# zovoilis-lab/Flye

Hardware: AMD Instinct MI355X
Metric: Gbp reads overlapped/sec (higher is better)
Workload: dtype u64

## Files before the change

### flye_amd/csrc/fg_chain.hip

```cpp
#include "fg_wavesort.h"

#include <algorithm>

#define WG 256
#define I32_MIN ((i32)0x80000000)

struct ChainParams {
	int k, maxJump, minOverlap, maxOverhang;
	int checkOverhang, forceLocal;
	float minUnique;
	u32 firstId;
	u32 qFirstId;
	int onlyMaxExt;
	int keepAln;
	int ablate;
	int lazy;
	unsigned long long* lazyCnt;
};

namespace {

struct CandAcc {
	typedef int4 T;
	int4* c;
	__device__ int4 load(int i) const { return c[i]; }
	__device__ void store(int i, const int4& x) { c[i] = x; }
	__device__ bool less(const int4& a, const int4& b) const { return a.w > b.w; }
};

__device__ __forceinline__ bool overlap_test(const ChainParams& P, u32 curId, u32 extId, i32 curLen,
											 i32 extLen, i32 cb, i32 ce, i32 eb, i32 ee)
{
	const i32 curRange = ce - cb, extRange = ee - eb;
	if (curRange < P.minOverlap || extRange < P.minOverlap) return false;
	const float lengthDiff = (float)abs(curRange - extRange);
	if (lengthDiff > 0.5f * (float)min(curRange, extRange)) return false;
	if (curId == extId)
	{
		const i32 inter = min(ce, ee) - max(cb, eb);
		if (inter > curRange / 2) return false;
	}
	if (curId == (extId ^ 1u))
	{
		const i32 inter = min(ce, extLen - eb) - max(cb, extLen - ee);
		if (inter > curRange / 2) return false;
	}
	if (!P.forceLocal && P.checkOverhang)
	{
		const i32 ovh = max(min(cb, eb), min(curLen - ce, extLen - ee));
		if (ovh > P.maxOverhang) return false;
	}
	return true;
}

#define LIST_ITEMS 8
__device__ __forceinline__ void append2_multi(const bool (&a)[LIST_ITEMS], const bool (&b)[LIST_ITEMS], u32 g0,
											  u32* listA, u32* listB, u32* counts)
{
	__shared__ u32 wtot[2][WG / 64];
	__shared__ u32 base[2];
	const int lane = threadIdx.x & 63, wv = threadIdx.x >> 6;
	u32 cA = 0, cB = 0;
#pragma unroll
	for (int t = 0; t < LIST_ITEMS; ++t) { cA += a[t]; cB += b[t]; }
	u32 iA = cA, iB = cB;
	for (int o = 1; o < 64; o <<= 1)
	{
		const u32 x = __shfl_up(iA, o), y = __shfl_up(iB, o);
		if (lane >= o) { iA += x; iB += y; }
	}
	if (lane == 63) { wtot[0][wv] = iA; wtot[1][wv] = iB; }
	__syncthreads();
	if (threadIdx.x < 2)
	{
		u32 t = 0;
		for (int i = 0; i < WG / 64; ++i) t += wtot[threadIdx.x][i];
		base[threadIdx.x] = t ? atomicAdd(&counts[threadIdx.x], t) : 0u;
	}
	__syncthreads();
	u32 oA = base[0] + iA - cA, oB = base[1] + iB - cB;
	for (int i = 0; i < wv; ++i) { oA += wtot[0][i]; oB += wtot[1][i]; }
#pragma unroll
	for (int t = 0; t < LIST_ITEMS; ++t)
	{
		if (a[t]) listA[oA++] = g0 + (u32)t;
		if (b[t]) listB[oB++] = g0 + (u32)t;
	}
}

__global__ void k_group_list(u64 nGroups, u64 nHits, const u64* __restrict__ groupStart, u32 minSize,
							 const u32* __restrict__ groupFirstCur, const u32* __restrict__ groupLastCur, i32 minOverlap,
							 u32* __restrict__ list, u32* __restrict__ listBig, u32 bigMin,
							 u32* __restrict__ listFused, u32 fusedMax , u32* __restrict__ counts,
							 u32* __restrict__ primCount, u32* __restrict__ dpSize)
{
	const u64 g0 = ((u64)blockIdx.x * WG + threadIdx.x) * LIST_ITEMS;
	bool a[LIST_ITEMS], b[LIST_ITEMS], f[LIST_ITEMS], none[LIST_ITEMS];
	u64 start = g0 < nGroups ? groupStart[g0] : nHits;
#pragma unroll
	for (int t = 0; t < LIST_ITEMS; ++t)
	{
		const u64 g = g0 + t;
		u64 n = 0;
		bool ok = false;
		if (g < nGroups)
		{
			primCount[g] = 0;
			dpSize[g] = 0;
			const u64 gend = (g + 1 < nGroups) ? groupStart[g + 1] : nHits;
			n = gend - start;
			if (n >= minSize && n > 0)
				ok = (i32)groupLastCur[g] - (i32)groupFirstCur[g] >= minOverlap;
			start = gend;
		}
		f[t] = ok && n <= fusedMax;
		a[t] = ok && n > fusedMax && n <= bigMin;
		b[t] = ok && n > bigMin && n > fusedMax;
		none[t] = false;
	}
	append2_multi(a, b, (u32)g0, list, listBig, counts);
	if (fusedMax)
	{
		__syncthreads();
		append2_multi(f, none, (u32)g0, listFused, listFused, counts + 2);
	}
}

#ifndef FIN_CAP_S
#define FIN_CAP_S 256
#endif
#ifndef FIN_CAP_M
#define FIN_CAP_M 1024
#endif
#ifndef FIN_WAVES_S
#define FIN_WAVES_S 1
#endif
#ifndef FIN_WAVES_G
#define FIN_WAVES_G 1
#endif
#ifndef FIN_BT_CAP
#define FIN_BT_CAP 1024
#endif
__global__ void k_dp_list(u64 nGroups, const u32* __restrict__ dpSize, u32 hugeMin, u32 doneMax ,
						  u32* __restrict__ listSmall, u32* __restrict__ listMid, u32* __restrict__ listBig, u32* __restrict__ counts)
{
	const u64 g0 = ((u64)blockIdx.x * WG + threadIdx.x) * LIST_ITEMS;
	bool a[LIST_ITEMS], b[LIST_ITEMS], h[LIST_ITEMS], none[LIST_ITEMS];
#pragma unroll
	for (int t = 0; t < LIST_ITEMS; ++t)
	{
		const u32 n = g0 + t < nGroups ? dpSize[g0 + t] : 0u;
		a[t] = n > doneMax && n <= FIN_CAP_S;
		b[t] = n > FIN_CAP_S && n > doneMax && n <= hugeMin;
		h[t] = n > hugeMin && n > FIN_CAP_S && n > doneMax;
		none[t] = false;
	}
	append2_multi(a, b, (u32)g0, listSmall, listMid, counts);
	__syncthreads();
	append2_multi(h, none, (u32)g0, listBig, listBig, counts + 2);
}

#ifndef PREP_CAP
#define PREP_CAP 320
#endif
#ifndef PREP_WAVES
#define PREP_WAVES 1
#endif
template <class KT>
__global__ void __launch_bounds__(PREP_WAVES * 64)
k_group_prep(ChainParams P, const u32* __restrict__ list, u32 nList, u64 nGroups, u64 nHits,
			 const u64* __restrict__ groupStart, const u32* __restrict__ groupQuery,
			 const u32* __restrict__ query, const i32* __restrict__ len, const i32* __restrict__ qLen,
			 HitKeyView<KT> hitKey, const u32* __restrict__ groupExt,
			 u32* __restrict__ gCur, u32* __restrict__ gExt, u32* __restrict__ gAux ,
			 u32* __restrict__ dpSize, uint8_t* __restrict__ groupExtSorted)
{
	__shared__ u32 sExt[PREP_WAVES][PREP_CAP];
// ... 197 lines not shown
				}
				const i32 j = jb - lane;
				i32 cp = FAR, ep = FAR, sj = 0;
				if (j >= 0)
				{
					if (WHOLE) { cp = (i32)cur[j]; ep = (i32)ext[j]; sj = score[j]; }
					else if (j >= tb0 - DP_RING)
					{
						cp = ringC[j & (DP_RING - 1)]; ep = ringE[j & (DP_RING - 1)]; sj = ringS[j & (DP_RING - 1)];
					}
					else
					{
						__builtin_amdgcn_s_waitcnt(0);
						cp = (i32)cur[j]; ep = (i32)ext[j];
						sj = __hip_atomic_load(&score[j], __ATOMIC_RELAXED, __HIP_MEMORY_SCOPE_AGENT);
					}
				}
				const i32 dc = cn - cp, de = en - ep;
				const bool inr = max((u32)(dc - 1), (u32)(de - 1)) < (u32)(maxJump - 1);
				const i32 jd = (i32)abs_diff(dc, de);
				i32 nsRaw = sj + min(min(dc, de), k) - (jd > 100 ? 2 * jd : (jd >> 1));
				asm volatile("" : "+v"(nsRaw));
				const i32 ns = inr ? nsRaw : I32_MIN;
				const u64 inrM = __builtin_amdgcn_ballot_w64(inr);
				const u64 mB = __builtin_amdgcn_ballot_w64((EXTS ? de : dc) > maxJump);
				const u64 mA = __builtin_amdgcn_ballot_w64(dc == de) & __builtin_amdgcn_ballot_w64(dc < k) & inrM;
				done = dp_scan_step(ns, mA, __popcll(~mB), jb, maxScore, maxId);
			}
			const i32 sNew = max(maxScore, k);
			ts = hl == il ? sNew + off : ts;
			tbk = lane == il ? (maxScore > k ? maxId : -1) : tbk;
		}
		asm volatile("" : "+v"(ntc), "+v"(nte));
		if (valid)
		{
			score[tb0 + lane] = ts; back[tb0 + lane] = tbk;
			if (!WHOLE) { ringC[(tb0 + lane) & (DP_RING - 1)] = tc; ringE[(tb0 + lane) & (DP_RING - 1)] = te; ringS[(tb0 + lane) & (DP_RING - 1)] = ts; }
		}
		if (WHOLE) wsort::wave_mem_fence();
		{
			const i32 tileMax = __builtin_amdgcn_readlane(wave_incl_max(valid ? ts : I32_MIN), 63);
			pmRun = max(pmRun, tileMax);
			const int t = tb0 >> 6;
			if (t < 64) pmv = lane == t ? pmRun : pmv;
		}
		pc = tc; pe = te; ps = ts;
	}
}

__global__ void __launch_bounds__(DP_WAVES * 64)
k_chain_dp(ChainParams P, const u32* __restrict__ list, u32 nList, u64 nGroups, u64 nHits,
		   const u64* __restrict__ groupStart, const u32* __restrict__ groupQuery,
		   const u32* __restrict__ query, const i32* __restrict__ len, const i32* __restrict__ qLen,
		   const uint8_t* __restrict__ groupExtSorted,
		   const u32* __restrict__ gCur, const u32* __restrict__ gExt,
		   i32* __restrict__ gScore, i32* __restrict__ gBack)
{
	const u32 li = blockIdx.x * DP_WAVES + (threadIdx.x >> 6);
	if (li >= nList) return;
	const u64 g = fg_uni(list[li]);
	const u64 g0 = fg_uni(groupStart[g]);
	const u64 gend = (g + 1 < nGroups) ? fg_uni(groupStart[g + 1]) : nHits;
	const i32 n = (i32)(gend - g0);
	const bool extSorted = fg_uni((u32)groupExtSorted[g]) != 0;
	__shared__ i32 ring[DP_WAVES][3][DP_RING];
	i32* ringC = ring[threadIdx.x >> 6][0];
	i32* ringE = ring[threadIdx.x >> 6][1];
	i32* ringS = ring[threadIdx.x >> 6][2];
	if (extSorted) dp_group<true>(P.k, P.maxJump, n, gCur + g0, gExt + g0, gScore + g0, gBack + g0, ringC, ringE, ringS);
	else dp_group<false>(P.k, P.maxJump, n, gCur + g0, gExt + g0, gScore + g0, gBack + g0, ringC, ringE, ringS);
}

template <int R>
__device__ __forceinline__ i32 fast_score_order(const i32 n, const i32* score, const i32* back, u32* oval)
{
	const int lane = threadIdx.x & 63;
	u32 v[R];
	bool wide = false;
#pragma unroll
	for (int r = 0; r < R; ++r)
	{
		const i32 e = r * 64 + lane;
		const bool live = e < n && back[e] != -1;
		const i32 sc = live ? score[e] : 0;
		wide |= live && (u32)sc >= (1u << 22);
		v[r] = live ? ((u32)((1 << 22) - 1 - sc) << 10) | (u32)e : 0xFFFFFFFFu;
	}
	if (__builtin_amdgcn_ballot_w64(wide)) return -1;
#pragma unroll
	for (int k = 2; k <= 64 * R; k <<= 1)
	{
#pragma unroll
		for (int j = k >> 1; j > 0; j >>= 1)
		{
			if (j >= 64)
			{
#pragma unroll
				for (int r = 0; r < R; ++r)
				{
					const int rp = r ^ (j >> 6);
					if (rp > r)
					{
						const bool asc = ((r * 64) & k) == 0;
						const u32 lo = min(v[r], v[rp]), hi = max(v[r], v[rp]);
						v[r] = asc ? lo : hi; v[rp] = asc ? hi : lo;
					}
				}
			}
			else
			{
#pragma unroll
				for (int r = 0; r < R; ++r)
				{
// ... 271 lines not shown
				m &= __builtin_amdgcn_ballot_w64(bk2 != -1);
			}
		}
	}
	wsort::wave_mem_fence();
	if (lane != 0) return;
	if (ncand == 0) return;
	if (ncand > 16)
	{
		CandAcc acc{cd};
		fgsort::sort(acc, 0, ncand, stack);
		best = cd[0];
	}
	if (P.onlyMaxExt)
	{
		cd[0] = best;
		*primCountG = 1;
		return;
	}
	if (ncand <= 16)
		for (i32 a = 1; a < ncand; ++a)
		{
			const int4 v = cd[a];
			i32 b = a - 1;
			while (b >= 0 && cd[b].w < v.w) { cd[b + 1] = cd[b]; --b; }
			cd[b + 1] = v;
		}
	i32 nprim = 0;
	for (i32 a = 0; a < ncand; ++a)
	{
		const int4 o = cd[a];
		const i32 ocb = (i32)cur[o.x], oce = (i32)cur[o.y], oeb = (i32)ext[o.x], oee = (i32)ext[o.y];
		bool contained = false;
		for (i32 b = 0; b < nprim && !contained; ++b)
		{
			const int4 pr = cd[b];
			contained = pr.w > o.w && (i32)cur[pr.x] <= ocb && oce <= (i32)cur[pr.y] &&
						(i32)ext[pr.x] <= oeb && oee <= (i32)ext[pr.y];
		}
		if (!contained) cd[nprim++] = o;
	}
	*primCountG = (u32)nprim;
}


template <int CAP, int FIN_WAVES, int BT_CAP = 0>
__global__ void __launch_bounds__(FIN_WAVES * 64)
k_chain_finish(ChainParams P, const u32* __restrict__ list, u32 nList, u64 nGroups, u64 nHits,
			   const u64* __restrict__ groupStart, const u32* __restrict__ groupQuery,
			   const u32* __restrict__ query, const i32* __restrict__ len, const i32* __restrict__ qLen,
			   const u32* __restrict__ groupExt,
			   const u32* __restrict__ gCur, const u32* __restrict__ gExt, i32* __restrict__ gScore,
			   i32* __restrict__ gBack, u32* __restrict__ gAux , int4* __restrict__ cand,
			   u32* __restrict__ primCount)
{
	constexpr bool USE_LDS = CAP > 0;
	extern __shared__ __attribute__((aligned(16))) char finLds[];
	__shared__ int stack[FIN_WAVES][3 * 40];
	__shared__ int small[FIN_WAVES][3 * 8];
	__shared__ i32 btLds[FIN_WAVES][BT_CAP > 0 ? BT_CAP : 1];
	const int wv = threadIdx.x >> 6;
	const int lane = threadIdx.x & 63;
	const u32 li = blockIdx.x * FIN_WAVES + wv;
	if (li >= nList) return;
	const u64 g = fg_uni(list[li]);
	const u64 g0 = fg_uni(groupStart[g]);
	const u64 gend = (g + 1 < nGroups) ? fg_uni(groupStart[g + 1]) : nHits;
	const i32 n = (i32)(gend - g0);
	const u32 q = groupQuery[g];
	const u32* cur = gCur + g0;
	const u32* ext = gExt + g0;
	i32 *score, *back; u32 *okey, *oval;
	unsigned short* plLds = nullptr;
	if (USE_LDS)
	{
		char* base = finLds + (size_t)wv * CAP * 20;
		score = (i32*)base; back = score + CAP; okey = (u32*)(back + CAP); oval = okey + CAP;
		plLds = (unsigned short*)(oval + CAP);
		for (i32 i = lane; i < n; i += 64) { score[i] = gScore[g0 + i]; back[i] = gBack[g0 + i]; }
		wsort::wave_mem_fence();
	}
	else
	{
		score = gScore + g0; back = gBack + g0; okey = gAux + 4 * g0; oval = okey + n;
	}
	const u32 qrec = query[q];
	const u32 extId = groupExt[g];
	finish_group<USE_LDS, BT_CAP>(P, n, P.qFirstId + qrec, extId, qLen[qrec >> 1], len[(extId - P.firstId) >> 1], cur, ext, score, back,
								  okey, oval, plLds, stack[wv], small[wv], btLds[wv], cand + g0, primCount + g);
}

template <class KT>
__global__ void __launch_bounds__(64)
k_chain_small(ChainParams P, const u32* __restrict__ list, u32 nList, u64 nGroups, u64 nHits,
			  const u64* __restrict__ groupStart, const u32* __restrict__ groupQuery,
			  const u32* __restrict__ query, const i32* __restrict__ len, const i32* __restrict__ qLen,
			  HitKeyView<KT> hitKey, const u32* __restrict__ groupExt,
			  u32* __restrict__ gCur, u32* __restrict__ gExt, i32* __restrict__ gBack, int4* __restrict__ cand,
			  u32* __restrict__ dpSize, u32* __restrict__ primCount, int cap )
{
	extern __shared__ __attribute__((aligned(16))) char smallLds[];
	u32* const sCur = (u32*)smallLds; u32* const sExt = sCur + cap;
	i32* const sScore = (i32*)(sExt + cap); i32* const sBack = sScore + cap;
	u32* const sOkey = (u32*)(sBack + cap); u32* const sOval = sOkey + cap;
	unsigned short* const sP = (unsigned short*)(sOval + cap);
	__shared__ int stack[3 * 40];
	__shared__ int small[3 * 8];
	const int lane = threadIdx.x;
	const u32 li = blockIdx.x;
	if (li >= nList) return;
	const u64 g = fg_uni(list[li]);
	const u64 g0 = fg_uni(groupStart[g]);
	const u64 gend = (g + 1 < nGroups) ? fg_uni(groupStart[g + 1]) : nHits;
	const i32 n = (i32)(gend - g0);
	const u32 qrec = query[groupQuery[g]];
	const u32 extId = groupExt[g];
	const i32 curLen = qLen[qrec >> 1];
	const i32 extLen = len[(extId - P.firstId) >> 1];
// ... 32 lines not shown
		if (__builtin_amdgcn_ballot_w64(!asc))
			wsort::wave_sort<u32, unsigned short>(sExt, sCur, n, sP, sP + n, stack, small);
	}
	for (i32 i = lane; i < n; i += 64) { gCur[g0 + i] = sCur[i]; gExt[g0 + i] = sExt[i]; }
	wsort::wave_mem_fence();
	if (extSorted) dp_group<true, true>(P.k, P.maxJump, n, sCur, sExt, sScore, sBack, nullptr, nullptr, nullptr);
	else dp_group<false, true>(P.k, P.maxJump, n, sCur, sExt, sScore, sBack, nullptr, nullptr, nullptr);
	wsort::wave_mem_fence();
	if (P.keepAln)
		for (i32 i = lane; i < n; i += 64) gBack[g0 + i] = sBack[i];
	finish_group<true, 0>(P, n, P.qFirstId + qrec, extId, curLen, extLen, sCur, sExt, sScore, sBack, sOkey, sOval, sP, stack, small,
						  nullptr, cand + g0, primCount + g);
}

u32 fetchU32(fg_ctx* c, const u32* dptr)
{
	u32 v;
	HIP_CHECK(hipMemcpyAsync(&v, dptr, 4, hipMemcpyDeviceToHost, c->stream));
	HIP_CHECK(hipStreamSynchronize(c->stream));
	return v;
}

}

u32 fgChainSmallMax()
{
	if (getenv("FG_CHAIN_FUSED") && atoi(getenv("FG_CHAIN_FUSED")) == 0) return 0u;
	return getenv("FG_FUSED_CAP") ? (u32)std::max(64, std::min(1024, atoi(getenv("FG_FUSED_CAP")))) : (u32)FIN_CAP_S;
}

void fgChainStage(fg_ctx* c, const fg_detector_params* p, uint8_t forceLocal, u64 nGroups, u64 nHits, int keyMode,
				  int curBits)
{
	hipStream_t s = c->stream;
	ChainParams cp;
	cp.k = c->k; cp.maxJump = p->max_jump; cp.minOverlap = p->min_overlap; cp.maxOverhang = p->max_overhang;
	cp.checkOverhang = p->max_overhang > 0; cp.forceLocal = forceLocal ? 1 : 0;
	{
		const float minKmerSruvivalRate = 0.01;
		cp.minUnique = minKmerSruvivalRate * p->min_overlap;
	}
	cp.firstId = c->firstId;
	cp.qFirstId = c->hasQ ? c->qFirstId : c->firstId;
	cp.onlyMaxExt = p->only_max_ext ? 1 : 0;
	cp.keepAln = p->keep_alignment ? 1 : 0;
	cp.ablate = getenv("FG_ABLATE") ? atoi(getenv("FG_ABLATE")) : 0;
	cp.lazy = cp.onlyMaxExt && !(getenv("FG_CHAIN_LAZY") && atoi(getenv("FG_CHAIN_LAZY")) == 0);
	cp.lazyCnt = c->dLazyCnt.p;
	if (!nGroups) return;
	const i32* qLen = c->hasQ ? c->dQLen.p : c->dLen.p;
	u32 minSize = 0;
	while ((float)minSize < cp.minUnique) ++minSize;
	if (minSize == 0) minSize = 1;
	c->dListSmall.reserve(nGroups + 1); c->dListBig.reserve(nGroups + 1); c->dListDp.reserve(nGroups + 1);
	c->dGroupExtSorted.reserve(nGroups + 1);
	c->dListCnt.reserve(4);
	const u64 hitCap = std::max<u64>(nHits, c->hitCapHint);
	c->dCur.reserve(hitCap + 16); c->dExt.reserve(hitCap + 16);
	c->dScore.reserve(hitCap + 16); c->dBack.reserve(hitCap + 16);
	c->dTmp32.reserve(4 * hitCap + 16);
	c->dCand.reserve(hitCap + 1);
	const unsigned gridG = (unsigned)((nGroups + (u64)WG * LIST_ITEMS - 1) / ((u64)WG * LIST_ITEMS));
	const u32 fusedMax = fgChainSmallMax();
	const bool fused = fusedMax != 0;
	if (fused) c->dListFused.reserve(nGroups + 1);
	HIP_CHECK(hipMemsetAsync(c->dListCnt.p, 0, 16, s));
	{ ScopedK t(c->timer, "k_group_list");
	  hipLaunchKernelGGL(k_group_list, gridG, WG, 0, s, nGroups, nHits, c->dGroupStart.p, minSize, c->dGroupFirstCur.p,
						 c->dGroupLastCur.p, (i32)p->min_overlap, c->dListSmall.p, c->dListBig.p, (u32)PREP_CAP,
						 c->dListFused.p, fusedMax, c->dListCnt.p, c->dPrimFlag.p, c->dDpSize.p); }
	u32 nPrep[4];
	c->hScalar.reserve(8);
	HIP_CHECK(hipMemcpyAsync(c->hScalar.p, c->dListCnt.p, 16, hipMemcpyDeviceToHost, s));
	HIP_CHECK(hipStreamSynchronize(s));
	memcpy(nPrep, c->hScalar.p, 16);
	const u32 nFused = fused ? nPrep[2] : 0u;
	if (!nPrep[0] && !nPrep[1] && !nFused) return;
	if (fused)
	{
		const bool others = nPrep[0] || nPrep[1];
		const bool sideStreams = !(getenv("FG_CHAIN_STREAMS") && atoi(getenv("FG_CHAIN_STREAMS")) == 1);
		if (others && sideStreams)
		{
			HIP_CHECK(hipEventRecord(c->evFork, s));
			HIP_CHECK(hipStreamWaitEvent(c->stream2, c->evFork, 0));
		}
		if (nFused)
		{
			ScopedK t(c->timer, "k_chain_small");
#define SMALL_ARGS(view) cp, c->dListFused.p, nFused, nGroups, nHits, c->dGroupStart.p, c->dGroupQuery.p, c->curQuery, c->dLen.p, qLen, \
			view, c->dGroupExt.p, c->dCur.p, c->dExt.p, c->dBack.p, c->dCand.p, c->dDpSize.p, c->dPrimFlag.p, (int)fusedMax
			const size_t ldsSmall = (size_t)fusedMax * 28;
			if (keyMode == 0)
				hipLaunchKernelGGL(k_chain_small<u32>, nFused, 64, ldsSmall, s, SMALL_ARGS((HitKeyView<u32>{c->dHitKey32.p, c->dHitVal.p, curBits, c->firstId})));
			else if (keyMode == 1)
				hipLaunchKernelGGL(k_chain_small<PK>, nFused, 64, ldsSmall, s, SMALL_ARGS((HitKeyView<PK>{(const PK*)c->dHitKey.p, nullptr, curBits, c->firstId})));
			else
				hipLaunchKernelGGL(k_chain_small<u64>, nFused, 64, ldsSmall, s, SMALL_ARGS((HitKeyView<u64>{c->dHitKey.p, c->dHitVal.p, curBits, c->firstId})));
#undef SMALL_ARGS
		}
		if (!others) return;
		hipStream_t s2 = sideStreams ? c->stream2 : s, s3 = sideStreams ? c->stream3 : s;
		const u32* prepList[2] = {c->dListSmall.p, c->dListBig.p};
#define PREP_ARGS(view, cls) cp, prepList[cls], nPrep[cls], nGroups, nHits, c->dGroupStart.p, c->dGroupQuery.p, c->curQuery, c->dLen.p, qLen, \
		view, c->dGroupExt.p, c->dCur.p, c->dExt.p, c->dTmp32.p, c->dDpSize.p, c->dGroupExtSorted.p
		for (int cls = 1; cls >= 0; --cls)
		{
			if (!nPrep[cls]) continue;
			ScopedK t(c->timer, "k_group_prep", s2);
			const unsigned gridP = (nPrep[cls] + PREP_WAVES - 1) / PREP_WAVES;
			if (keyMode == 0)
				hipLaunchKernelGGL(k_group_prep<u32>, gridP, PREP_WAVES * 64, 0, s2,
								   PREP_ARGS((HitKeyView<u32>{c->dHitKey32.p, c->dHitVal.p, curBits, c->firstId}), cls));
			else if (keyMode == 1)
				hipLaunchKernelGGL(k_group_prep<PK>, gridP, PREP_WAVES * 64, 0, s2,
								   PREP_ARGS((HitKeyView<PK>{(const PK*)c->dHitKey.p, nullptr, curBits, c->firstId}), cls));
			else
				hipLaunchKernelGGL(k_group_prep<u64>, gridP, PREP_WAVES * 64, 0, s2,
								   PREP_ARGS((HitKeyView<u64>{c->dHitKey.p, c->dHitVal.p, curBits, c->firstId}), cls));
		}
#undef PREP_ARGS
		HIP_CHECK(hipMemsetAsync(c->dListCnt.p, 0, 16, s2));
		const bool smallCall2 = (nPrep[0] + nPrep[1] + nFused) < 65536u && !getenv("FG_CHAIN_NO_SMALL_CALL");
		const u32 hugeMin2 = getenv("FG_CHAIN_HUGE_MIN") ? (u32)atoi(getenv("FG_CHAIN_HUGE_MIN")) : (smallCall2 ? (u32)FIN_CAP_M : 4096u);
		{ ScopedK t(c->timer, "k_dp_list", s2);
		  hipLaunchKernelGGL(k_dp_list, gridG, WG, 0, s2, nGroups, c->dDpSize.p, hugeMin2, fusedMax, c->dListSmall.p, c->dListDp.p,
							 c->dListBig.p, c->dListCnt.p); }
		u32 hc2[4];
		HIP_CHECK(hipMemcpyAsync(c->hScalar.p, c->dListCnt.p, 16, hipMemcpyDeviceToHost, s2));
		HIP_CHECK(hipStreamSynchronize(s2));
		memcpy(hc2, c->hScalar.p, 16);
		const u32* lists2[3] = {c->dListSmall.p, c->dListDp.p, c->dListBig.p};
		if (hc2[2] && sideStreams)
		{
			HIP_CHECK(hipEventRecord(c->evJoin3, s2));
			HIP_CHECK(hipStreamWaitEvent(s3, c->evJoin3, 0));
		}
#define FIN_ARGS2(cls) cp, lists2[cls], hc2[cls], nGroups, nHits, c->dGroupStart.p, c->dGroupQuery.p, c->curQuery, c->dLen.p, \
		qLen, c->dGroupExt.p, c->dCur.p, c->dExt.p, c->dScore.p, c->dBack.p, c->dTmp32.p, c->dCand.p, c->dPrimFlag.p
#define DP_ARGS2(cls) cp, lists2[cls], hc2[cls], nGroups, nHits, c->dGroupStart.p, c->dGroupQuery.p, c->curQuery, c->dLen.p, qLen, \
		c->dGroupExtSorted.p, c->dCur.p, c->dExt.p, c->dScore.p, c->dBack.p
		for (int cls = 2; cls >= 1; --cls)
		{
			if (!hc2[cls]) continue;
			hipStream_t on = cls == 2 ? s3 : s2;
			{ ScopedK t(c->timer, "k_chain_dp", on);
			  hipLaunchKernelGGL(k_chain_dp, (hc2[cls] + DP_WAVES - 1) / DP_WAVES, DP_WAVES * 64, 0, on, DP_ARGS2(cls)); }
			if (cls == 1 && smallCall2 && hugeMin2 <= (u32)FIN_CAP_M)
			{
				ScopedK t(c->timer, "k_chain_finish<lds1024>", on);
				hipLaunchKernelGGL((k_chain_finish<FIN_CAP_M, 1>), hc2[cls], 64, FIN_CAP_M * 20, on, FIN_ARGS2(cls));
			}
			else
			{
				ScopedK t(c->timer, "k_chain_finish<global>", on);
				hipLaunchKernelGGL((k_chain_finish<0, FIN_WAVES_G, FIN_BT_CAP>), (hc2[cls] + FIN_WAVES_G - 1) / FIN_WAVES_G, FIN_WAVES_G * 64, 0, on,
								   FIN_ARGS2(cls));
			}
		}
		if (hc2[0])
		{
			{ ScopedK t(c->timer, "k_chain_dp", s2);
			  hipLaunchKernelGGL(k_chain_dp, (hc2[0] + DP_WAVES - 1) / DP_WAVES, DP_WAVES * 64, 0, s2, DP_ARGS2(0)); }
			{ ScopedK t(c->timer, "k_chain_finish<lds256>", s2);
			  hipLaunchKernelGGL((k_chain_finish<FIN_CAP_S, FIN_WAVES_S>), (hc2[0] + FIN_WAVES_S - 1) / FIN_WAVES_S, FIN_WAVES_S * 64,
								 FIN_CAP_S * 20 * FIN_WAVES_S, s2, FIN_ARGS2(0)); }
		}
#undef DP_ARGS2
#undef FIN_ARGS2
		if (sideStreams)
		{
			HIP_CHECK(hipEventRecord(c->evJoin, s2));
			HIP_CHECK(hipStreamWaitEvent(s, c->evJoin, 0));
			if (hc2[2])
			{
				HIP_CHECK(hipEventRecord(c->evJoin3, s3));
				HIP_CHECK(hipStreamWaitEvent(s, c->evJoin3, 0));
			}
		}
		return;
	}
	const bool twoStreams = !(getenv("FG_CHAIN_STREAMS") && atoi(getenv("FG_CHAIN_STREAMS")) == 1);
	auto fork = [&](bool both) -> hipStream_t
	{
		if (!twoStreams || !both) return s;
		HIP_CHECK(hipEventRecord(c->evFork, s));
		HIP_CHECK(hipStreamWaitEvent(c->stream2, c->evFork, 0));
		return c->stream2;
	};
	auto join = [&](hipStream_t side)
	{
		if (side == s) return;
		HIP_CHECK(hipEventRecord(c->evJoin, side));
		HIP_CHECK(hipStreamWaitEvent(s, c->evJoin, 0));
	};
	{
		hipStream_t sBig = fork(nPrep[0] && nPrep[1]);
		const u32* prepList[2] = {c->dListSmall.p, c->dListBig.p};
#define PREP_ARGS(view, cls) cp, prepList[cls], nPrep[cls], nGroups, nHits, c->dGroupStart.p, c->dGroupQuery.p, c->curQuery, c->dLen.p, qLen, \
		view, c->dGroupExt.p, c->dCur.p, c->dExt.p, c->dTmp32.p, c->dDpSize.p, c->dGroupExtSorted.p
		for (int cls = 1; cls >= 0; --cls)
		{
			if (!nPrep[cls]) continue;
			hipStream_t on = cls ? sBig : s;
			ScopedK t(c->timer, "k_group_prep", on);
			const unsigned gridP = (nPrep[cls] + PREP_WAVES - 1) / PREP_WAVES;
			if (keyMode == 0)
				hipLaunchKernelGGL(k_group_prep<u32>, gridP, PREP_WAVES * 64, 0, on,
								   PREP_ARGS((HitKeyView<u32>{c->dHitKey32.p, c->dHitVal.p, curBits, c->firstId}), cls));
			else if (keyMode == 1)
				hipLaunchKernelGGL(k_group_prep<PK>, gridP, PREP_WAVES * 64, 0, on,
								   PREP_ARGS((HitKeyView<PK>{(const PK*)c->dHitKey.p, nullptr, curBits, c->firstId}), cls));
			else
				hipLaunchKernelGGL(k_group_prep<u64>, gridP, PREP_WAVES * 64, 0, on,
								   PREP_ARGS((HitKeyView<u64>{c->dHitKey.p, c->dHitVal.p, curBits, c->firstId}), cls));
		}
#undef PREP_ARGS
		join(sBig);
	}
	HIP_CHECK(hipMemsetAsync(c->dListCnt.p, 0, 16, s));
	const bool smallCall = (nPrep[0] + nPrep[1]) < 65536u && !getenv("FG_CHAIN_NO_SMALL_CALL");
	const u32 hugeMin = getenv("FG_CHAIN_HUGE_MIN") ? (u32)atoi(getenv("FG_CHAIN_HUGE_MIN")) : (smallCall ? (u32)FIN_CAP_M : 4096u);
	{ ScopedK t(c->timer, "k_dp_list");
	  hipLaunchKernelGGL(k_dp_list, gridG, WG, 0, s, nGroups, c->dDpSize.p, hugeMin, 0u, c->dListSmall.p, c->dListDp.p,
						 c->dListBig.p, c->dListCnt.p); }
	u32 hc[4];
	HIP_CHECK(hipMemcpyAsync(c->hScalar.p, c->dListCnt.p, 16, hipMemcpyDeviceToHost, s));
	HIP_CHECK(hipStreamSynchronize(s));
	memcpy(hc, c->hScalar.p, 16);
	const u32* lists[3] = {c->dListSmall.p, c->dListDp.p, c->dListBig.p};
	const bool side = twoStreams && hc[0] && (hc[1] || hc[2]);
	hipStream_t sMid = s, sHuge = s;
	if (side)
	{
		HIP_CHECK(hipEventRecord(c->evFork, s));
		HIP_CHECK(hipStreamWaitEvent(c->stream2, c->evFork, 0));
		HIP_CHECK(hipStreamWaitEvent(c->stream3, c->evFork, 0));
		sMid = c->stream2; sHuge = c->stream3;
	}
#define FIN_ARGS(cls) cp, lists[cls], hc[cls], nGroups, nHits, c->dGroupStart.p, c->dGroupQuery.p, c->curQuery, c->dLen.p, \
		qLen, c->dGroupExt.p, c->dCur.p, c->dExt.p, c->dScore.p, c->dBack.p, c->dTmp32.p, c->dCand.p, c->dPrimFlag.p
#define DP_ARGS(cls) cp, lists[cls], hc[cls], nGroups, nHits, c->dGroupStart.p, c->dGroupQuery.p, c->curQuery, c->dLen.p, qLen, \
		c->dGroupExtSorted.p, c->dCur.p, c->dExt.p, c->dScore.p, c->dBack.p
	for (int cls = 2; cls >= 1; --cls)
	{
		if (!hc[cls]) continue;
		hipStream_t on = cls == 2 ? sHuge : sMid;
		{ ScopedK t(c->timer, "k_chain_dp", on);
		  hipLaunchKernelGGL(k_chain_dp, (hc[cls] + DP_WAVES - 1) / DP_WAVES, DP_WAVES * 64, 0, on, DP_ARGS(cls)); }
		if (cls == 1 && smallCall && hugeMin <= (u32)FIN_CAP_M)
		{
			ScopedK t(c->timer, "k_chain_finish<lds1024>", on);
			hipLaunchKernelGGL((k_chain_finish<FIN_CAP_M, 1>), hc[cls], 64, FIN_CAP_M * 20, on, FIN_ARGS(cls));
		}
		else
		{
			ScopedK t(c->timer, "k_chain_finish<global>", on);
			hipLaunchKernelGGL((k_chain_finish<0, FIN_WAVES_G, FIN_BT_CAP>), (hc[cls] + FIN_WAVES_G - 1) / FIN_WAVES_G, FIN_WAVES_G * 64, 0, on,
							   FIN_ARGS(cls));
		}
	}
	if (hc[0])
	{
		{ ScopedK t(c->timer, "k_chain_dp");
		  hipLaunchKernelGGL(k_chain_dp, (hc[0] + DP_WAVES - 1) / DP_WAVES, DP_WAVES * 64, 0, s, DP_ARGS(0)); }
		{ ScopedK t(c->timer, "k_chain_finish<lds256>");
		  hipLaunchKernelGGL((k_chain_finish<FIN_CAP_S, FIN_WAVES_S>), (hc[0] + FIN_WAVES_S - 1) / FIN_WAVES_S, FIN_WAVES_S * 64,
							 FIN_CAP_S * 20 * FIN_WAVES_S, s, FIN_ARGS(0)); }
	}
	if (side)
	{
		HIP_CHECK(hipEventRecord(c->evJoin, c->stream2));
		HIP_CHECK(hipStreamWaitEvent(s, c->evJoin, 0));
		HIP_CHECK(hipEventRecord(c->evJoin3, c->stream3));
		HIP_CHECK(hipStreamWaitEvent(s, c->evJoin3, 0));
	}
#undef DP_ARGS
#undef FIN_ARGS
}
```

Baseline: 4.773.

## Classify chain groups into mid/huge lists up front and drop second list pass

New measurement: 4.958 (median of 6 runs). +3.9%, better.

```diff
diff --git a/flye_amd/csrc/fg_chain.hip b/flye_amd/csrc/fg_chain.hip
--- a/flye_amd/csrc/fg_chain.hip
+++ b/flye_amd/csrc/fg_chain.hip
@@ -54,8 +54,8 @@
 }
 
 #define LIST_ITEMS 8
-__device__ __forceinline__ void append2_multi(const bool (&a)[LIST_ITEMS], const bool (&b)[LIST_ITEMS], u32 g0,
-											  u32* listA, u32* listB, u32* counts)
+__device__ __forceinline__ void append2_offsets(const bool (&a)[LIST_ITEMS], const bool (&b)[LIST_ITEMS], u32* counts,
+												u32& oA, u32& oB)
 {
 	__shared__ u32 wtot[2][WG / 64];
 	__shared__ u32 base[2];
@@ -78,8 +78,14 @@
 		base[threadIdx.x] = t ? atomicAdd(&counts[threadIdx.x], t) : 0u;
 	}
 	__syncthreads();
-	u32 oA = base[0] + iA - cA, oB = base[1] + iB - cB;
+	oA = base[0] + iA - cA; oB = base[1] + iB - cB;
 	for (int i = 0; i < wv; ++i) { oA += wtot[0][i]; oB += wtot[1][i]; }
+}
+__device__ __forceinline__ void append2_multi(const bool (&a)[LIST_ITEMS], const bool (&b)[LIST_ITEMS], u32 g0,
+											  u32* listA, u32* listB, u32* counts)
+{
+	u32 oA, oB;
+	append2_offsets(a, b, counts, oA, oB);
 #pragma unroll
 	for (int t = 0; t < LIST_ITEMS; ++t)
 	{
@@ -88,14 +94,15 @@
 	}
 }
 
+template <bool CLASSES>
 __global__ void k_group_list(u64 nGroups, u64 nHits, const u64* __restrict__ groupStart, u32 minSize,
 							 const u32* __restrict__ groupFirstCur, const u32* __restrict__ groupLastCur, i32 minOverlap,
-							 u32* __restrict__ list, u32* __restrict__ listBig, u32 bigMin,
+							 u32* __restrict__ list, u32* __restrict__ listBig, u32 bigMin, u32 hugeMax, u32 mid,
 							 u32* __restrict__ listFused, u32 fusedMax , u32* __restrict__ counts,
 							 u32* __restrict__ primCount, u32* __restrict__ dpSize)
 {
 	const u64 g0 = ((u64)blockIdx.x * WG + threadIdx.x) * LIST_ITEMS;
-	bool a[LIST_ITEMS], b[LIST_ITEMS], f[LIST_ITEMS], none[LIST_ITEMS];
+	bool a[LIST_ITEMS], b[LIST_ITEMS], f[LIST_ITEMS], m[LIST_ITEMS];
 	u64 start = g0 < nGroups ? groupStart[g0] : nHits;
 #pragma unroll
 	for (int t = 0; t < LIST_ITEMS; ++t)
@@ -116,13 +123,31 @@
 		f[t] = ok && n <= fusedMax;
 		a[t] = ok && n > fusedMax && n <= bigMin;
 		b[t] = ok && n > bigMin && n > fusedMax;
-		none[t] = false;
-	}
-	append2_multi(a, b, (u32)g0, list, listBig, counts);
-	if (fusedMax)
-	{
-		__syncthreads();
-		append2_multi(f, none, (u32)g0, listFused, listFused, counts + 2);
+		m[t] = false;
+		if (CLASSES) { m[t] = b[t] && n <= hugeMax; b[t] = b[t] && !m[t]; }
+	}
+	if (!CLASSES)
+	{
+		append2_multi(a, b, (u32)g0, list, listBig, counts);
+		if (fusedMax)
+		{
+			__syncthreads();
+			append2_multi(f, m, (u32)g0, listFused, listFused, counts + 2);
+		}
+		return;
+	}
+	u32 oA, oB, oF, oM;
+	append2_offsets(a, b, counts, oA, oB);
+	__syncthreads();
+	append2_offsets(f, m, counts + 2, oF, oM);
+#pragma unroll
+	for (int t = 0; t < LIST_ITEMS; ++t)
+	{
+		const u32 g = (u32)g0 + (u32)t;
+		if (a[t]) list[(size_t)mid - 1 - oA++] = g;
+		if (b[t]) listBig[(size_t)mid - 1 - oB++] = g;
+		if (f[t]) listFused[oF++] = g;
+		if (m[t]) { list[(size_t)mid + oM] = g; listBig[(size_t)mid + oM] = g; ++oM; }
 	}
 }
 
@@ -426,13 +451,14 @@
 k_chain_dp(ChainParams P, const u32* __restrict__ list, u32 nList, u64 nGroups, u64 nHits,
 		   const u64* __restrict__ groupStart, const u32* __restrict__ groupQuery,
 		   const u32* __restrict__ query, const i32* __restrict__ len, const i32* __restrict__ qLen,
-		   const uint8_t* __restrict__ groupExtSorted,
+		   const uint8_t* __restrict__ groupExtSorted, const u32* __restrict__ dpSize,
 		   const u32* __restrict__ gCur, const u32* __restrict__ gExt,
 		   i32* __restrict__ gScore, i32* __restrict__ gBack)
 {
 	const u32 li = blockIdx.x * DP_WAVES + (threadIdx.x >> 6);
 	if (li >= nList) return;
 	const u64 g = fg_uni(list[li]);
+	if (fg_uni(dpSize[g]) == 0) return;
 	const u64 g0 = fg_uni(groupStart[g]);
 	const u64 gend = (g + 1 < nGroups) ? fg_uni(groupStart[g + 1]) : nHits;
 	const i32 n = (i32)(gend - g0);
@@ -810,7 +836,7 @@
 			   const u32* __restrict__ groupExt,
 			   const u32* __restrict__ gCur, const u32* __restrict__ gExt, i32* __restrict__ gScore,
 			   i32* __restrict__ gBack, u32* __restrict__ gAux , int4* __restrict__ cand,
-			   u32* __restrict__ primCount)
+			   u32* __restrict__ primCount, const u32* __restrict__ dpSize)
 {
 	constexpr bool USE_LDS = CAP > 0;
 	extern __shared__ __attribute__((aligned(16))) char finLds[];
@@ -822,6 +848,7 @@
 	const u32 li = blockIdx.x * FIN_WAVES + wv;
 	if (li >= nList) return;
 	const u64 g = fg_uni(list[li]);
+	if (fg_uni(dpSize[g]) == 0) return;
 	const u64 g0 = fg_uni(groupStart[g]);
 	const u64 gend = (g + 1 < nGroups) ? fg_uni(groupStart[g + 1]) : nHits;
 	const i32 n = (i32)(gend - g0);
@@ -960,7 +987,11 @@
 	u32 minSize = 0;
 	while ((float)minSize < cp.minUnique) ++minSize;
 	if (minSize == 0) minSize = 1;
-	c->dListSmall.reserve(nGroups + 1); c->dListBig.reserve(nGroups + 1); c->dListDp.reserve(nGroups + 1);
+	const u32 fusedMax = fgChainSmallMax();
+	const bool fused = fusedMax != 0;
+	const bool classes = fusedMax >= (u32)FIN_CAP_S;
+	c->dListBig.reserve((classes ? 2 : 1) * nGroups + 1); c->dListDp.reserve((classes ? 2 : 1) * nGroups + 1);
+	if (!classes) c->dListSmall.reserve(nGroups + 1);
 	c->dGroupExtSorted.reserve(nGroups + 1);
 	c->dListCnt.reserve(4);
 	const u64 hitCap = std::max<u64>(nHits, c->hitCapHint);
@@ -969,175 +1000,147 @@
 	c->dTmp32.reserve(4 * hitCap + 16);
 	c->dCand.reserve(hitCap + 1);
 	const unsigned gridG = (unsigned)((nGroups + (u64)WG * LIST_ITEMS - 1) / ((u64)WG * LIST_ITEMS));
-	const u32 fusedMax = fgChainSmallMax();
-	const bool fused = fusedMax != 0;
 	if (fused) c->dListFused.reserve(nGroups + 1);
+	const char* hugeEnv = getenv("FG_CHAIN_HUGE_MIN");
 	HIP_CHECK(hipMemsetAsync(c->dListCnt.p, 0, 16, s));
 	{ ScopedK t(c->timer, "k_group_list");
-	  hipLaunchKernelGGL(k_group_list, gridG, WG, 0, s, nGroups, nHits, c->dGroupStart.p, minSize, c->dGroupFirstCur.p,
-						 c->dGroupLastCur.p, (i32)p->min_overlap, c->dListSmall.p, c->dListBig.p, (u32)PREP_CAP,
-						 c->dListFused.p, fusedMax, c->dListCnt.p, c->dPrimFlag.p, c->dDpSize.p); }
+	  if (classes)
+		  hipLaunchKernelGGL(k_group_list<true>, gridG, WG, 0, s, nGroups, nHits, c->dGroupStart.p, minSize, c->dGroupFirstCur.p,
+							 c->dGroupLastCur.p, (i32)p->min_overlap, c->dListDp.p, c->dListBig.p,
+							 hugeEnv ? (u32)atoi(hugeEnv) : (u32)FIN_CAP_M, hugeEnv ? (u32)atoi(hugeEnv) : 4096u, (u32)nGroups,
+							 c->dListFused.p, fusedMax, c->dListCnt.p, c->dPrimFlag.p, c->dDpSize.p);
+	  else
+		  hipLaunchKernelGGL(k_group_list<false>, gridG, WG, 0, s, nGroups, nHits, c->dGroupStart.p, minSize, c->dGroupFirstCur.p,
+							 c->dGroupLastCur.p, (i32)p->min_overlap, c->dListSmall.p, c->dListBig.p, (u32)PREP_CAP, 0u, 0u,
+							 c->dListFused.p, fusedMax, c->dListCnt.p, c->dPrimFlag.p, c->dDpSize.p); }
 	u32 nPrep[4];
 	c->hScalar.reserve(8);
 	HIP_CHECK(hipMemcpyAsync(c->hScalar.p, c->dListCnt.p, 16, hipMemcpyDeviceToHost, s));
 	HIP_CHECK(hipStreamSynchronize(s));
 	memcpy(nPrep, c->hScalar.p, 16);
 	const u32 nFused = fused ? nPrep[2] : 0u;
-	if (!nPrep[0] && !nPrep[1] && !nFused) return;
-	if (fused)
-	{
-		const bool others = nPrep[0] || nPrep[1];
-		const bool sideStreams = !(getenv("FG_CHAIN_STREAMS") && atoi(getenv("FG_CHAIN_STREAMS")) == 1);
-		if (others && sideStreams)
+	if (!nPrep[0] && !nPrep[1] && !nPrep[3] && !nFused) return;
+	const bool sideStreams = !(getenv("FG_CHAIN_STREAMS") && atoi(getenv("FG_CHAIN_STREAMS")) == 1);
+	auto launchSmall = [&]()
+	{
+		if (!nFused) return;
+		ScopedK t(c->timer, "k_chain_small");
+#define SMALL_ARGS(view) cp, c->dListFused.p, nFused, nGroups, nHits, c->dGroupStart.p, c->dGroupQuery.p, c->curQuery, c->dLen.p, qLen, \
+		view, c->dGroupExt.p, c->dCur.p, c->dExt.p, c->dBack.p, c->dCand.p, c->dDpSize.p, c->dPrimFlag.p, (int)fusedMax
+		const size_t ldsSmall = (size_t)fusedMax * 28;
+		if (keyMode == 0)
+			hipLaunchKernelGGL(k_chain_small<u32>, nFused, 64, ldsSmall, s, SMALL_ARGS((HitKeyView<u32>{c->dHitKey32.p, c->dHitVal.p, curBits, c->firstId})));
+		else if (keyMode == 1)
+			hipLaunchKernelGGL(k_chain_small<PK>, nFused, 64, ldsSmall, s, SMALL_ARGS((HitKeyView<PK>{(const PK*)c->dHitKey.p, nullptr, curBits, c->firstId})));
+		else
+			hipLaunchKernelGGL(k_chain_small<u64>, nFused, 64, ldsSmall, s, SMALL_ARGS((HitKeyView<u64>{c->dHitKey.p, c->dHitVal.p, curBits, c->firstId})));
+#undef SMALL_ARGS
+	};
+	auto launchPrep = [&](const u32* list, u32 nList, hipStream_t on)
+	{
+		ScopedK t(c->timer, "k_group_prep", on);
+#define PREP_ARGS(view) cp, list, nList, nGroups, nHits, c->dGroupStart.p, c->dGroupQuery.p, c->curQuery, c->dLen.p, qLen, \
+		view, c->dGroupExt.p, c->dCur.p, c->dExt.p, c->dTmp32.p, c->dDpSize.p, c->dGroupExtSorted.p
+		const unsigned gridP = (nList + PREP_WAVES - 1) / PREP_WAVES;
+		if (keyMode == 0)
+			hipLaunchKernelGGL(k_group_prep<u32>, gridP, PREP_WAVES * 64, 0, on,
+							   PREP_ARGS((HitKeyView<u32>{c->dHitKey32.p, c->dHitVal.p, curBits, c->firstId})));
+		else if (keyMode == 1)
+			hipLaunchKernelGGL(k_group_prep<PK>, gridP, PREP_WAVES * 64, 0, on,
+							   PREP_ARGS((HitKeyView<PK>{(const PK*)c->dHitKey.p, nullptr, curBits, c->firstId})));
+		else
+			hipLaunchKernelGGL(k_group_prep<u64>, gridP, PREP_WAVES * 64, 0, on,
+							   PREP_ARGS((HitKeyView<u64>{c->dHitKey.p, c->dHitVal.p, curBits, c->firstId})));
+#undef PREP_ARGS
+	};
+#define FIN_ARGS(list, n) cp, list, n, nGroups, nHits, c->dGroupStart.p, c->dGroupQuery.p, c->curQuery, c->dLen.p, \
+		qLen, c->dGroupExt.p, c->dCur.p, c->dExt.p, c->dScore.p, c->dBack.p, c->dTmp32.p, c->dCand.p, c->dPrimFlag.p, c->dDpSize.p
+#define DP_ARGS(list, n) cp, list, n, nGroups, nHits, c->dGroupStart.p, c->dGroupQuery.p, c->curQuery, c->dLen.p, qLen, \
+		c->dGroupExtSorted.p, c->dDpSize.p, c->dCur.p, c->dExt.p, c->dScore.p, c->dBack.p
+	if (classes)
+	{
+		const bool smallCall = (nPrep[0] + nPrep[1] + nPrep[3] + nFused) < 65536u && !getenv("FG_CHAIN_NO_SMALL_CALL");
+		const u32 nMid = nPrep[0] + (smallCall ? 0u : nPrep[3]), nHuge = nPrep[1] + (smallCall ? nPrep[3] : 0u);
+		const u32* listMid = c->dListDp.p + (nGroups - nPrep[0]);
+		const u32* listHuge = c->dListBig.p + (nGroups - nPrep[1]);
+		const bool midLds = smallCall && (!hugeEnv || (u32)atoi(hugeEnv) <= (u32)FIN_CAP_M);
+		const bool side = sideStreams && (nMid || nHuge);
+		hipStream_t sMid = side ? c->stream2 : s, sHuge = side ? c->stream3 : s;
+		const bool split = side && !smallCall && !nHuge && !(getenv("FG_CHAIN_SPLIT") && atoi(getenv("FG_CHAIN_SPLIT")) == 0);
+		const u32 nMidB = split ? nMid / 2 : 0u, nMidA = nMid - nMidB;
+		auto chain = [&](const u32* list, u32 n, hipStream_t on, bool lds)
+		{
+			if (!n) return;
+			launchPrep(list, n, on);
+			{ ScopedK t(c->timer, "k_chain_dp", on);
+			  hipLaunchKernelGGL(k_chain_dp, (n + DP_WAVES - 1) / DP_WAVES, DP_WAVES * 64, 0, on, DP_ARGS(list, n)); }
+			if (lds)
+			{
+				ScopedK t(c->timer, "k_chain_finish<lds1024>", on);
+				hipLaunchKernelGGL((k_chain_finish<FIN_CAP_M, 1>), n, 64, FIN_CAP_M * 20, on, FIN_ARGS(list, n));
+			}
+			else
+			{
+				ScopedK t(c->timer, "k_chain_finish<global>", on);
+				hipLaunchKernelGGL((k_chain_finish<0, FIN_WAVES_G, FIN_BT_CAP>), (n + FIN_WAVES_G - 1) / FIN_WAVES_G, FIN_WAVES_G * 64, 0, on,
+								   FIN_ARGS(list, n));
+			}
+		};
+		if (side)
+		{
+			HIP_CHECK(hipEventRecord(c->evFork, s));
+			if (nMidA) HIP_CHECK(hipStreamWaitEvent(sMid, c->evFork, 0));
+			if (nHuge || nMidB) HIP_CHECK(hipStreamWaitEvent(sHuge, c->evFork, 0));
+		}
+		chain(listHuge, nHuge, sHuge, false);
+		chain(listMid, nMidA, sMid, midLds);
+		chain(listMid + nMidA, nMidB, sHuge, midLds);
+		launchSmall();
+		if (side)
+		{
+			if (nMidA)
+			{
+				HIP_CHECK(hipEventRecord(c->evJoin, sMid));
+				HIP_CHECK(hipStreamWaitEvent(s, c->evJoin, 0));
+			}
+			if (nHuge || nMidB)
+			{
+				HIP_CHECK(hipEventRecord(c->evJoin3, sHuge));
+				HIP_CHECK(hipStreamWaitEvent(s, c->evJoin3, 0));
+			}
+		}
+		return;
+	}
+	launchSmall();
+	if (!nPrep[0] && !nPrep[1]) return;
+	{
+		hipStream_t sBig = s;
+		if (sideStreams && nPrep[0] && nPrep[1])
 		{
 			HIP_CHECK(hipEventRecord(c->evFork, s));
 			HIP_CHECK(hipStreamWaitEvent(c->stream2, c->evFork, 0));
-		}
-		if (nFused)
-		{
-			ScopedK t(c->timer, "k_chain_small");
-#define SMALL_ARGS(view) cp, c->dListFused.p, nFused, nGroups, nHits, c->dGroupStart.p, c->dGroupQuery.p, c->curQuery, c->dLen.p, qLen, \
-			view, c->dGroupExt.p, c->dCur.p, c->dExt.p, c->dBack.p, c->dCand.p, c->dDpSize.p, c->dPrimFlag.p, (int)fusedMax
-			const size_t ldsSmall = (size_t)fusedMax * 28;
-			if (keyMode == 0)
-				hipLaunchKernelGGL(k_chain_small<u32>, nFused, 64, ldsSmall, s, SMALL_ARGS((HitKeyView<u32>{c->dHitKey32.p, c->dHitVal.p, curBits, c->firstId})));
-			else if (keyMode == 1)
-				hipLaunchKernelGGL(k_chain_small<PK>, nFused, 64, ldsSmall, s, SMALL_ARGS((HitKeyView<PK>{(const PK*)c->dHitKey.p, nullptr, curBits, c->firstId})));
-			else
-				hipLaunchKernelGGL(k_chain_small<u64>, nFused, 64, ldsSmall, s, SMALL_ARGS((HitKeyView<u64>{c->dHitKey.p, c->dHitVal.p, curBits, c->firstId})));
-#undef SMALL_ARGS
-		}
-		if (!others) return;
-		hipStream_t s2 = sideStreams ? c->stream2 : s, s3 = sideStreams ? c->stream3 : s;
-		const u32* prepList[2] = {c->dListSmall.p, c->dListBig.p};
-#define PREP_ARGS(view, cls) cp, prepList[cls], nPrep[cls], nGroups, nHits, c->dGroupStart.p, c->dGroupQuery.p, c->curQuery, c->dLen.p, qLen, \
-		view, c->dGroupExt.p, c->dCur.p, c->dExt.p, c->dTmp32.p, c->dDpSize.p, c->dGroupExtSorted.p
-		for (int cls = 1; cls >= 0; --cls)
-		{
-			if (!nPrep[cls]) continue;
-			ScopedK t(c->timer, "k_group_prep", s2);
-			const unsigned gridP = (nPrep[cls] + PREP_WAVES - 1) / PREP_WAVES;
-			if (keyMode == 0)
-				hipLaunchKernelGGL(k_group_prep<u32>, gridP, PREP_WAVES * 64, 0, s2,
-								   PREP_ARGS((HitKeyView<u32>{c->dHitKey32.p, c->dHitVal.p, curBits, c->firstId}), cls));
-			else if (keyMode == 1)
-				hipLaunchKernelGGL(k_group_prep<PK>, gridP, PREP_WAVES * 64, 0, s2,
-								   PREP_ARGS((HitKeyView<PK>{(const PK*)c->dHitKey.p, nullptr, curBits, c->firstId}), cls));
-			else
-				hipLaunchKernelGGL(k_group_prep<u64>, gridP, PREP_WAVES * 64, 0, s2,
-								   PREP_ARGS((HitKeyView<u64>{c->dHitKey.p, c->dHitVal.p, curBits, c->firstId}), cls));
-		}
-#undef PREP_ARGS
-		HIP_CHECK(hipMemsetAsync(c->dListCnt.p, 0, 16, s2));
-		const bool smallCall2 = (nPrep[0] + nPrep[1] + nFused) < 65536u && !getenv("FG_CHAIN_NO_SMALL_CALL");
-		const u32 hugeMin2 = getenv("FG_CHAIN_HUGE_MIN") ? (u32)atoi(getenv("FG_CHAIN_HUGE_MIN")) : (smallCall2 ? (u32)FIN_CAP_M : 4096u);
-		{ ScopedK t(c->timer, "k_dp_list", s2);
-		  hipLaunchKernelGGL(k_dp_list, gridG, WG, 0, s2, nGroups, c->dDpSize.p, hugeMin2, fusedMax, c->dListSmall.p, c->dListDp.p,
-							 c->dListBig.p, c->dListCnt.p); }
-		u32 hc2[4];
-		HIP_CHECK(hipMemcpyAsync(c->hScalar.p, c->dListCnt.p, 16, hipMemcpyDeviceToHost, s2));
-		HIP_CHECK(hipStreamSynchronize(s2));
-		memcpy(hc2, c->hScalar.p, 16);
-		const u32* lists2[3] = {c->dListSmall.p, c->dListDp.p, c->dListBig.p};
-		if (hc2[2] && sideStreams)
-		{
-			HIP_CHECK(hipEventRecord(c->evJoin3, s2));
-			HIP_CHECK(hipStreamWaitEvent(s3, c->evJoin3, 0));
-		}
-#define FIN_ARGS2(cls) cp, lists2[cls], hc2[cls], nGroups, nHits, c->dGroupStart.p, c->dGroupQuery.p, c->curQuery, c->dLen.p, \
-		qLen, c->dGroupExt.p, c->dCur.p, c->dExt.p, c->dScore.p, c->dBack.p, c->dTmp32.p, c->dCand.p, c->dPrimFlag.p
-#define DP_ARGS2(cls) cp, lists2[cls], hc2[cls], nGroups, nHits, c->dGroupStart.p, c->dGroupQuery.p, c->curQuery, c->dLen.p, qLen, \
-		c->dGroupExtSorted.p, c->dCur.p, c->dExt.p, c->dScore.p, c->dBack.p
-		for (int cls = 2; cls >= 1; --cls)
-		{
-			if (!hc2[cls]) continue;
-			hipStream_t on = cls == 2 ? s3 : s2;
-			{ ScopedK t(c->timer, "k_chain_dp", on);
-			  hipLaunchKernelGGL(k_chain_dp, (hc2[cls] + DP_WAVES - 1) / DP_WAVES, DP_WAVES * 64, 0, on, DP_ARGS2(cls)); }
-			if (cls == 1 && smallCall2 && hugeMin2 <= (u32)FIN_CAP_M)
-			{
-				ScopedK t(c->timer, "k_chain_finish<lds1024>", on);
-				hipLaunchKernelGGL((k_chain_finish<FIN_CAP_M, 1>), hc2[cls], 64, FIN_CAP_M * 20, on, FIN_ARGS2(cls));
-			}
-			else
-			{
-				ScopedK t(c->timer, "k_chain_finish<global>", on);
-				hipLaunchKernelGGL((k_chain_finish<0, FIN_WAVES_G, FIN_BT_CAP>), (hc2[cls] + FIN_WAVES_G - 1) / FIN_WAVES_G, FIN_WAVES_G * 64, 0, on,
-								   FIN_ARGS2(cls));
-			}
-		}
-		if (hc2[0])
-		{
-			{ ScopedK t(c->timer, "k_chain_dp", s2);
-			  hipLaunchKernelGGL(k_chain_dp, (hc2[0] + DP_WAVES - 1) / DP_WAVES, DP_WAVES * 64, 0, s2, DP_ARGS2(0)); }
-			{ ScopedK t(c->timer, "k_chain_finish<lds256>", s2);
-			  hipLaunchKernelGGL((k_chain_finish<FIN_CAP_S, FIN_WAVES_S>), (hc2[0] + FIN_WAVES_S - 1) / FIN_WAVES_S, FIN_WAVES_S * 64,
-								 FIN_CAP_S * 20 * FIN_WAVES_S, s2, FIN_ARGS2(0)); }
-		}
-#undef DP_ARGS2
-#undef FIN_ARGS2
-		if (sideStreams)
-		{
-			HIP_CHECK(hipEventRecord(c->evJoin, s2));
+			sBig = c->stream2;
+		}
+		if (nPrep[1]) launchPrep(c->dListBig.p, nPrep[1], sBig);
+		if (nPrep[0]) launchPrep(c->dListSmall.p, nPrep[0], s);
+		if (sBig != s)
+		{
+			HIP_CHECK(hipEventRecord(c->evJoin, sBig));
 			HIP_CHECK(hipStreamWaitEvent(s, c->evJoin, 0));
-			if (hc2[2])
-			{
-				HIP_CHECK(hipEventRecord(c->evJoin3, s3));
-				HIP_CHECK(hipStreamWaitEvent(s, c->evJoin3, 0));
-			}
-		}
-		return;
-	}
-	const bool twoStreams = !(getenv("FG_CHAIN_STREAMS") && atoi(getenv("FG_CHAIN_STREAMS")) == 1);
-	auto fork = [&](bool both) -> hipStream_t
-	{
-		if (!twoStreams || !both) return s;
-		HIP_CHECK(hipEventRecord(c->evFork, s));
-		HIP_CHECK(hipStreamWaitEvent(c->stream2, c->evFork, 0));
-		return c->stream2;
-	};
-	auto join = [&](hipStream_t side)
-	{
-		if (side == s) return;
-		HIP_CHECK(hipEventRecord(c->evJoin, side));
-		HIP_CHECK(hipStreamWaitEvent(s, c->evJoin, 0));
-	};
-	{
-		hipStream_t sBig = fork(nPrep[0] && nPrep[1]);
-		const u32* prepList[2] = {c->dListSmall.p, c->dListBig.p};
-#define PREP_ARGS(view, cls) cp, prepList[cls], nPrep[cls], nGroups, nHits, c->dGroupStart.p, c->dGroupQuery.p, c->curQuery, c->dLen.p, qLen, \
-		view, c->dGroupExt.p, c->dCur.p, c->dExt.p, c->dTmp32.p, c->dDpSize.p, c->dGroupExtSorted.p
-		for (int cls = 1; cls >= 0; --cls)
-		{
-			if (!nPrep[cls]) continue;
-			hipStream_t on = cls ? sBig : s;
-			ScopedK t(c->timer, "k_group_prep", on);
-			const unsigned gridP = (nPrep[cls] + PREP_WAVES - 1) / PREP_WAVES;
-			if (keyMode == 0)
-				hipLaunchKernelGGL(k_group_prep<u32>, gridP, PREP_WAVES * 64, 0, on,
-								   PREP_ARGS((HitKeyView<u32>{c->dHitKey32.p, c->dHitVal.p, curBits, c->firstId}), cls));
-			else if (keyMode == 1)
-				hipLaunchKernelGGL(k_group_prep<PK>, gridP, PREP_WAVES * 64, 0, on,
-								   PREP_ARGS((HitKeyView<PK>{(const PK*)c->dHitKey.p, nullptr, curBits, c->firstId}), cls));
-			else
-				hipLaunchKernelGGL(k_group_prep<u64>, gridP, PREP_WAVES * 64, 0, on,
-								   PREP_ARGS((HitKeyView<u64>{c->dHitKey.p, c->dHitVal.p, curBits, c->firstId}), cls));
-		}
-#undef PREP_ARGS
-		join(sBig);
+		}
 	}
 	HIP_CHECK(hipMemsetAsync(c->dListCnt.p, 0, 16, s));
-	const bool smallCall = (nPrep[0] + nPrep[1]) < 65536u && !getenv("FG_CHAIN_NO_SMALL_CALL");
-	const u32 hugeMin = getenv("FG_CHAIN_HUGE_MIN") ? (u32)atoi(getenv("FG_CHAIN_HUGE_MIN")) : (smallCall ? (u32)FIN_CAP_M : 4096u);
+	const bool smallCall = (nPrep[0] + nPrep[1] + nFused) < 65536u && !getenv("FG_CHAIN_NO_SMALL_CALL");
+	const u32 hugeMin = hugeEnv ? (u32)atoi(hugeEnv) : (smallCall ? (u32)FIN_CAP_M : 4096u);
 	{ ScopedK t(c->timer, "k_dp_list");
-	  hipLaunchKernelGGL(k_dp_list, gridG, WG, 0, s, nGroups, c->dDpSize.p, hugeMin, 0u, c->dListSmall.p, c->dListDp.p,
+	  hipLaunchKernelGGL(k_dp_list, gridG, WG, 0, s, nGroups, c->dDpSize.p, hugeMin, fusedMax, c->dListSmall.p, c->dListDp.p,
 						 c->dListBig.p, c->dListCnt.p); }
 	u32 hc[4];
 	HIP_CHECK(hipMemcpyAsync(c->hScalar.p, c->dListCnt.p, 16, hipMemcpyDeviceToHost, s));
 	HIP_CHECK(hipStreamSynchronize(s));
 	memcpy(hc, c->hScalar.p, 16);
 	const u32* lists[3] = {c->dListSmall.p, c->dListDp.p, c->dListBig.p};
-	const bool side = twoStreams && hc[0] && (hc[1] || hc[2]);
+	const bool side = sideStreams && hc[0] && (hc[1] || hc[2]);
 	hipStream_t sMid = s, sHuge = s;
 	if (side)
 	{
@@ -1146,35 +1149,31 @@
 		HIP_CHECK(hipStreamWaitEvent(c->stream3, c->evFork, 0));
 		sMid = c->stream2; sHuge = c->stream3;
 	}
-#define FIN_ARGS(cls) cp, lists[cls], hc[cls], nGroups, nHits, c->dGroupStart.p, c->dGroupQuery.p, c->curQuery, c->dLen.p, \
-		qLen, c->dGroupExt.p, c->dCur.p, c->dExt.p, c->dScore.p, c->dBack.p, c->dTmp32.p, c->dCand.p, c->dPrimFlag.p
-#define DP_ARGS(cls) cp, lists[cls], hc[cls], nGroups, nHits, c->dGroupStart.p, c->dGroupQuery.p, c->curQuery, c->dLen.p, qLen, \
-		c->dGroupExtSorted.p, c->dCur.p, c->dExt.p, c->dScore.p, c->dBack.p
 	for (int cls = 2; cls >= 1; --cls)
 	{
 		if (!hc[cls]) continue;
 		hipStream_t on = cls == 2 ? sHuge : sMid;
 		{ ScopedK t(c->timer, "k_chain_dp", on);
-		  hipLaunchKernelGGL(k_chain_dp, (hc[cls] + DP_WAVES - 1) / DP_WAVES, DP_WAVES * 64, 0, on, DP_ARGS(cls)); }
+		  hipLaunchKernelGGL(k_chain_dp, (hc[cls] + DP_WAVES - 1) / DP_WAVES, DP_WAVES * 64, 0, on, DP_ARGS(lists[cls], hc[cls])); }
 		if (cls == 1 && smallCall && hugeMin <= (u32)FIN_CAP_M)
 		{
 			ScopedK t(c->timer, "k_chain_finish<lds1024>", on);
-			hipLaunchKernelGGL((k_chain_finish<FIN_CAP_M, 1>), hc[cls], 64, FIN_CAP_M * 20, on, FIN_ARGS(cls));
+			hipLaunchKernelGGL((k_chain_finish<FIN_CAP_M, 1>), hc[cls], 64, FIN_CAP_M * 20, on, FIN_ARGS(lists[cls], hc[cls]));
 		}
 		else
 		{
 			ScopedK t(c->timer, "k_chain_finish<global>", on);
 			hipLaunchKernelGGL((k_chain_finish<0, FIN_WAVES_G, FIN_BT_CAP>), (hc[cls] + FIN_WAVES_G - 1) / FIN_WAVES_G, FIN_WAVES_G * 64, 0, on,
-							   FIN_ARGS(cls));
+							   FIN_ARGS(lists[cls], hc[cls]));
 		}
 	}
 	if (hc[0])
 	{
 		{ ScopedK t(c->timer, "k_chain_dp");
-		  hipLaunchKernelGGL(k_chain_dp, (hc[0] + DP_WAVES - 1) / DP_WAVES, DP_WAVES * 64, 0, s, DP_ARGS(0)); }
+		  hipLaunchKernelGGL(k_chain_dp, (hc[0] + DP_WAVES - 1) / DP_WAVES, DP_WAVES * 64, 0, s, DP_ARGS(lists[0], hc[0])); }
 		{ ScopedK t(c->timer, "k_chain_finish<lds256>");
 		  hipLaunchKernelGGL((k_chain_finish<FIN_CAP_S, FIN_WAVES_S>), (hc[0] + FIN_WAVES_S - 1) / FIN_WAVES_S, FIN_WAVES_S * 64,
-							 FIN_CAP_S * 20 * FIN_WAVES_S, s, FIN_ARGS(0)); }
+							 FIN_CAP_S * 20 * FIN_WAVES_S, s, FIN_ARGS(lists[0], hc[0])); }
 	}
 	if (side)
 	{
```
